# SheffieldML/GPy

Hardware: AMD Instinct MI355X
Metric: exact-GP log_lik+grad iters/sec (higher is better)
Workload: dtype f64; 1 GPU; BASELINE configs[2]: matern52 ARD exact GP, one GPRegression.parameters_changed, N=16384 D=32 Dy=1 per GPU; N=16384, D=32, kernel=matern52, ARD=True, parallelism=replicas x1

## Files before the change

### gpy_amd/csrc/kern.hip

```cpp
#include <cstdint>
#include <cstdlib>

#include "../../include/mi355gp.h"
#include "internal.h"

#define KT 64
#define KDC 32

struct CovVal {
    double k;
    double dk_r;
    double dk_or;
};

__device__ __forceinline__ double cov_k(int kind, double var, double r2, bool same = false) {
    if (kind == MI355GP_WHITE) return same ? var : 0.0;
    if (kind == MI355GP_BIAS) return var;
    if (kind == MI355GP_RBF) return var * exp(-0.5 * r2);
    const double r = sqrt(r2);
    if (kind == MI355GP_MATERN52) {
        const double s5r = 2.2360679774997896964 * r;
        return var * (1.0 + s5r + (5.0 / 3.0) * r2) * exp(-s5r);
    }
    if (kind == MI355GP_MATERN32) {
// ... 35 lines not shown
        return c;
    }
    c.k = var * exp(-r);
    c.dk_r = -r * c.k;
    c.dk_or = (r != 0.0) ? -c.k / r : 0.0;
    return c;
}

__global__ void k_scale_inputs(const double* __restrict__ X, long n, int D, const double* __restrict__ inv_ls,
                               int ard, double* __restrict__ Xt, long ldx) {
    const long idx = (long)blockIdx.x * blockDim.x + threadIdx.x;
    if (idx >= (long)D * ldx) return;
    const int q = (int)(idx / ldx);
    const long i = idx - (long)q * ldx;
    Xt[idx] = (i < n) ? X[i * D + q] * inv_ls[ard ? q : 0] : 0.0;
}

void launch_scale_inputs(hipStream_t st, const double* X, long n, int D, const double* inv_ls, int ard,
                         double* Xt, long ldx) {
    const long total = (long)D * ldx;
    hipLaunchKernelGGL(k_scale_inputs, dim3((unsigned)((total + 255) / 256)), dim3(256), 0, st, X, n, D, inv_ls,
                       ard, Xt, ldx);
}

__device__ __forceinline__ void stage_x(const double* __restrict__ Xt, long ldx, long i0, int q0, int qc,
                                        double* s, int t) {
    for (int idx = t; idx < qc * KT; idx += 256) {
        const int q = idx >> 6, ii = idx & 63;
        s[q * KT + ii] = Xt[(long)(q0 + q) * ldx + i0 + ii];
    }
}

#define KTJ 72
__device__ __forceinline__ int xj_pos(int ii) { return 40 * ((ii >> 1) & 1) + 2 * (ii >> 2) + (ii & 1); }
__device__ __forceinline__ void stage_xj(const double* __restrict__ Xt, long ldx, long i0, int q0, int qc, double* s, int t) {
    for (int idx = t; idx < qc * KT; idx += 256) {
        const int q = idx >> 6, ii = idx & 63;
        s[q * KTJ + xj_pos(ii)] = Xt[(long)(q0 + q) * ldx + i0 + ii];
    }
}
__device__ __forceinline__ d4 ld_xj(const double* sj, int q, int tx) {
    const d2 lo = *reinterpret_cast<const d2*>(sj + q * KTJ + 2 * tx);
    const d2 hi = *reinterpret_cast<const d2*>(sj + q * KTJ + 40 + 2 * tx);
    return d4{lo[0], lo[1], hi[0], hi[1]};
}

__device__ __forceinline__ void accum_r2(const double* si, const double* sj, int qc, int ty, int tx,
                                         double (&r2)[4][4]) {
    for (int q = 0; q < qc; ++q) {
        const d4 xi = *reinterpret_cast<const d4*>(si + q * KT + ty * 4);
        const d4 xj = ld_xj(sj, q, tx);
#pragma unroll
        for (int a = 0; a < 4; ++a)
#pragma unroll
            for (int b = 0; b < 4; ++b) {
                const double d = xi[a] - xj[b];
                r2[a][b] = fma(d, d, r2[a][b]);
            }
    }
}

template <bool SYM>
__global__ __launch_bounds__(256) void k_kbuild(KernParams kp, const double* __restrict__ Xt1, long ld1, long n,
                                                const double* __restrict__ Xt2, long ld2, long m,
                                                double* __restrict__ out, long ldo, long nrows_out,
                                                const double* __restrict__ noise, long noise_len, double jit,
                                                int lower_only, int add_diag, int ntc, int accumulate, int diag_same,
                                                const double* mul) {
    __shared__ __attribute__((aligned(16))) double si[KDC * KT];
    __shared__ __attribute__((aligned(16))) double sj[KDC * KTJ];
    const int t = threadIdx.x, tx = t & 15, ty = t >> 4;
    const long ti = blockIdx.x / ntc, tj = blockIdx.x % ntc;
    if (SYM && lower_only && tj > ti) return;
    const long i0 = ti * KT, j0 = tj * KT;
    double r2[4][4];
#pragma unroll
    for (int a = 0; a < 4; ++a)
#pragma unroll
        for (int b = 0; b < 4; ++b) r2[a][b] = 0.0;
    const bool real_tile = (i0 < n) && (j0 < m);
    if (real_tile) {
        for (int q0 = 0; q0 < kp.D; q0 += KDC) {
            const int qc = (kp.D - q0 < KDC) ? (kp.D - q0) : KDC;
            __syncthreads();
            stage_x(Xt1, ld1, i0, q0, qc, si, t);
            stage_xj(Xt2, ld2, j0, q0, qc, sj, t);
            __syncthreads();
            accum_r2(si, sj, qc, ty, tx, r2);
        }
    }
#pragma unroll
    for (int a = 0; a < 4; ++a) {
        const long i = i0 + ty * 4 + a;
        double v[4];
#pragma unroll
        for (int b = 0; b < 4; ++b) {
            const long j = j0 + tx * 4 + b;
            if (i < n && j < m) v[b] = cov_k(kp.kind, kp.variance, r2[a][b], (SYM || diag_same) && i == j);
            else v[b] = (SYM && i == j && !accumulate) ? 1.0 : 0.0;
        }
        if (SYM) {
            if (i < nrows_out) {
                d4* p = reinterpret_cast<d4*>(out + i * ldo + j0 + tx * 4);
                d4 o = (d4){v[0], v[1], v[2], v[3]};
                if (mul) o *= *reinterpret_cast<const d4*>(mul + i * ldo + j0 + tx * 4);
                if (add_diag && i < n) {
                    const long d = i - (j0 + tx * 4);
                    if (d >= 0 && d < 4) o[d] += noise[noise_len > 1 ? i : 0] + jit;
                }
                if (accumulate) o += *p;
                *p = o;
            }
        } else if (i < n) {
#pragma unroll
            for (int b = 0; b < 4; ++b) {
                const long j = j0 + tx * 4 + b;
                if (j < m) {
                    const double w = mul ? v[b] * mul[i * ldo + j] : v[b];
                    out[i * ldo + j] = accumulate ? out[i * ldo + j] + w : w;
                }
            }
        }
    }
}



#define KBC_DY 4
__global__ __launch_bounds__(256) void k_kbuild_cols(KernParams kp, const double* __restrict__ Xt1, long ld1, long n,
                                                     const double* __restrict__ Xt2, long ld2, long m, double* __restrict__ out,
                                                     long ldo, const double* __restrict__ V, int Dy, int ntc, int ntr,
                                                     int tiles_per_split, double* __restrict__ colpart, long mcols) {
    __shared__ __attribute__((aligned(16))) double si[KDC * KT];
    __shared__ __attribute__((aligned(16))) double sj[KDC * KTJ];
    __shared__ double sv[KT * KBC_DY];
    __shared__ double red[256];
    const int t = threadIdx.x, tx = t & 15, ty = t >> 4;
    const int tj = blockIdx.x % ntc, split = blockIdx.x / ntc;
    const long j0 = (long)tj * KT;
    const int D = kp.D;
    double csum[4][KBC_DY];
#pragma unroll
    for (int b = 0; b < 4; ++b)
#pragma unroll
        for (int d = 0; d < KBC_DY; ++d) csum[b][d] = 0.0;
    stage_xj(Xt2, ld2, j0, 0, D, sj, t);
    const bool fullcols = j0 + KT <= m;
    const int ti_end = ((split + 1) * tiles_per_split < ntr) ? (split + 1) * tiles_per_split : ntr;
    for (int ti = split * tiles_per_split; ti < ti_end; ++ti) {
        const long i0 = (long)ti * KT;
        __syncthreads();
        stage_x(Xt1, ld1, i0, 0, D, si, t);
        if (t < KT * Dy) {
            const long i = i0 + t / Dy;
            sv[(t / Dy) * KBC_DY + t % Dy] = (i < n) ? V[i * Dy + t % Dy] : 0.0;
        }
        __syncthreads();
        double r2[4][4];
#pragma unroll
        for (int a = 0; a < 4; ++a)
#pragma unroll
            for (int b = 0; b < 4; ++b) r2[a][b] = 0.0;
        accum_r2(si, sj, D, ty, tx, r2);
#pragma unroll
        for (int a = 0; a < 4; ++a) {
            const long i = i0 + ty * 4 + a;
            d4 o;
#pragma unroll
            for (int b = 0; b < 4; ++b) o[b] = (i < n && j0 + tx * 4 + b < m) ? cov_k(kp.kind, kp.variance, r2[a][b], false) : 0.0;
            if (i < n) {
                if (fullcols) *reinterpret_cast<d4*>(out + i * ldo + j0 + tx * 4) = o;
                else
#pragma unroll
                    for (int b = 0; b < 4; ++b)
                        if (j0 + tx * 4 + b < m) out[i * ldo + j0 + tx * 4 + b] = o[b];
            }
#pragma unroll
            for (int d = 0; d < KBC_DY; ++d) {
                if (d < Dy) {
                    const double v = sv[(ty * 4 + a) * KBC_DY + d];
#pragma unroll
                    for (int b = 0; b < 4; ++b) csum[b][d] = fma(o[b], v, csum[b][d]);
                }
            }
        }
    }
    double* cp = colpart + (long)split * mcols * Dy;
#pragma unroll
    for (int d = 0; d < KBC_DY; ++d) {
        if (d < Dy) {
#pragma unroll
            for (int b = 0; b < 4; ++b) {
                __syncthreads();
                red[ty * 16 + tx] = csum[b][d];
                __syncthreads();
                if (ty == 0) {
                    double sacc = 0.0;
                    for (int r = 0; r < 16; ++r) sacc += red[r * 16 + tx];
                    const long j = j0 + tx * 4 + b;
                    if (j < mcols) cp[j * Dy + d] = sacc;
                }
            }
        }
    }
}

int launch_kbuild_cols(hipStream_t st, KernParams kp, const double* Xt1, long ld1, long n, const double* Xt2, long ld2, long m,
                       long mcols, double* Kout, long ldk, const double* V, int Dy, double* colpart) {
    if (kp.D > KDC || kp.kind > MI355GP_EXPONENTIAL || Dy > KBC_DY || Dy < 1 || ldk % 4 != 0 || ((uintptr_t)Kout & 31) != 0) return 0;
    const int ntr = (int)((n + KT - 1) / KT), ntc = (int)((mcols + KT - 1) / KT);
    int nsplit = 2048 / ntc;
    if (nsplit > 64) nsplit = 64;
    if (nsplit > ntr) nsplit = ntr;
    if (nsplit < 1) nsplit = 1;
    const int tps = (ntr + nsplit - 1) / nsplit;
    nsplit = (ntr + tps - 1) / tps;
    hipLaunchKernelGGL(k_kbuild_cols, dim3((unsigned)(ntc * nsplit)), dim3(256), 0, st, kp, Xt1, ld1, n, Xt2, ld2, m, Kout, ldk, V, Dy,
                       ntc, ntr, tps, colpart, mcols);
    return nsplit;
}

static void launch_kbuild_ext(hipStream_t st, bool sym, KernParams kp, const double* Xt1, long ld1, long n, const double* Xt2,
                              long ld2, long m, double* out, long ldo, long nrows_out, const double* noise, long noise_len,
                              double jit, int lower_only, int add_diag, int ntc, int nblocks, int accumulate, int diag_same,
                              const double* mul);
static void launch_grad_ext(hipStream_t st, bool fused, KernParams kp, const double* Xt1, long ld1, long n, const double* Xt2,
                            long ld2, long m, const double* G, long ldg, const double* alpha, int Dy, long ntiles, int ntc,
                            double* partials, double* Hout, long ldh, const double* aa_scale, const double* Mul, long ldm);
static void launch_kbuild_coreg(hipStream_t st, bool sym, KernParams kp, const double* Xt1, long ld1, long n, const double* Xt2,
                                long ld2, long m, double* out, long ldo, long nrows_out, const double* noise, long noise_len,
                                double jit, int lower_only, int add_diag, int ntc, int nblocks, int accumulate, const double* mul);

static void launch_kbuild_lin(hipStream_t st, bool sym, KernParams kp, const double* Xt1, long ld1, long n, const double* Xt2,
                              long ld2, long m, double* out, long ldo, long nrows_out, const double* noise, long noise_len,
                              double jit, int lower_only, int add_diag, int ntc, int nblocks, int accumulate, const double* mul);
static void launch_grad_lin(hipStream_t st, bool fused, KernParams kp, const double* Xt1, long ld1, long n, const double* Xt2,
                            long ld2, long m, const double* G, long ldg, const double* alpha, int Dy, long ntiles, int ntc,
                            double* partials, double* Hout, long ldh, const double* aa_scale, const double* Mul, long ldm);

static inline bool dot_kind(int kind) { return kind == MI355GP_MLP || kind == MI355GP_POLY; }
static void launch_kbuild_dot(hipStream_t st, bool sym, KernParams kp, const double* Xt1, long ld1, long n, const double* Xt2,
                              long ld2, long m, double* out, long ldo, long nrows_out, const double* noise, long noise_len,
                              double jit, int lower_only, int add_diag, int ntc, int nblocks, int accumulate, const double* mul);
static void launch_grad_dot(hipStream_t st, bool fused, KernParams kp, const double* Xt1, long ld1, long n, const double* Xt2,
                            long ld2, long m, const double* G, long ldg, const double* alpha, int Dy, long ntiles, int ntc,
                            double* partials, double* Hout, long ldh, const double* aa_scale, const double* Mul, long ldm);

void launch_kbuild_sym(hipStream_t st, KernParams kp, const double* Xt, long ldx, long n, long npad, double* A,
                       const double* noise, long noise_len, double jit, int lower_only, int add_diag, int accumulate,
                       const double* mul) {
    const int nt = (int)(npad / KT);
    if (dot_kind(kp.kind)) {
        launch_kbuild_dot(st, true, kp, Xt, ldx, n, Xt, ldx, n, A, npad, npad, noise, noise_len, jit, lower_only, add_diag, nt,
                          nt * nt, accumulate, mul);
        return;
    }
    if (kp.kind == MI355GP_LINEAR) {
        launch_kbuild_lin(st, true, kp, Xt, ldx, n, Xt, ldx, n, A, npad, npad, noise, noise_len, jit, lower_only, add_diag, nt,
                          nt * nt, accumulate, mul);
        return;
    }
    if (kp.kind == MI355GP_COREGIONALIZE) {
        launch_kbuild_coreg(st, true, kp, Xt, ldx, n, Xt, ldx, n, A, npad, npad, noise, noise_len, jit, lower_only, add_diag, nt,
                            nt * nt, accumulate, mul);
        return;
    }
    if (kp.kind >= MI355GP_RATQUAD) {
        launch_kbuild_ext(st, true, kp, Xt, ldx, n, Xt, ldx, n, A, npad, npad, noise, noise_len, jit, lower_only, add_diag, nt,
                          nt * nt, accumulate, 0, mul);
        return;
    }
    hipLaunchKernelGGL((k_kbuild<true>), dim3((unsigned)((long)nt * nt)), dim3(256), 0, st, kp, Xt, ldx, n, Xt, ldx, n,
                       A, npad, npad, noise, noise_len, jit, lower_only, add_diag, nt, accumulate, 0, mul);
}

void launch_kbuild_cross(hipStream_t st, KernParams kp, const double* Xt1, long ld1, long n, const double* Xt2,
                         long ld2, long m, double* Kout, long ldk, int accumulate, int diag_same, const double* mul) {
    const int ntr = (int)((n + KT - 1) / KT), ntc = (int)((m + KT - 1) / KT);
    if (dot_kind(kp.kind)) {
        launch_kbuild_dot(st, false, kp, Xt1, ld1, n, Xt2, ld2, m, Kout, ldk, n, nullptr, 0, 0.0, 0, 0, ntc, ntr * ntc, accumulate,
                          mul);
        return;
    }
    if (kp.kind == MI355GP_LINEAR) {
        launch_kbuild_lin(st, false, kp, Xt1, ld1, n, Xt2, ld2, m, Kout, ldk, n, nullptr, 0, 0.0, 0, 0, ntc, ntr * ntc, accumulate,
                          mul);
        return;
    }
    if (kp.kind == MI355GP_COREGIONALIZE) {
        launch_kbuild_coreg(st, false, kp, Xt1, ld1, n, Xt2, ld2, m, Kout, ldk, n, nullptr, 0, 0.0, 0, 0, ntc, ntr * ntc, accumulate,
                            mul);
        return;
    }
    if (kp.kind >= MI355GP_RATQUAD) {
        launch_kbuild_ext(st, false, kp, Xt1, ld1, n, Xt2, ld2, m, Kout, ldk, n, nullptr, 0, 0.0, 0, 0, ntc, ntr * ntc,
                          accumulate, diag_same, mul);
        return;
    }
    hipLaunchKernelGGL((k_kbuild<false>), dim3((unsigned)((long)ntr * ntc)), dim3(256), 0, st, kp, Xt1, ld1, n, Xt2,
                       ld2, m, Kout, ldk, n, nullptr, 0, 0.0, 0, 0, ntc, accumulate, diag_same, mul);
}

#define GP_STRIDE 34
template <bool FUSED, bool ARD>
__global__ __launch_bounds__(256) void k_grad(KernParams kp, const double* __restrict__ Xt1, long ld1, long n,
                                              const double* __restrict__ Xt2, long ld2, long m,
                                              const double* __restrict__ G, long ldg,
                                              const double* __restrict__ alpha, int Dy, int q_off,
                                              long ntiles, int ntc, double* __restrict__ partials,
                                              double* __restrict__ Hout = nullptr, long ldh = 0, int diag_same = 0,
                                              const double* __restrict__ aa_scale = nullptr,
                                              const double* __restrict__ Mul = nullptr, long ldm = 0,
                                              RankTerm rk = RankTerm{nullptr, nullptr, 0, 0.0, 1.0, nullptr}) {
    __shared__ __attribute__((aligned(16))) double si[KDC * KT];
    __shared__ __attribute__((aligned(16))) double sj[KDC * KTJ];
    __shared__ double red[256];
    const int t = threadIdx.x, tx = t & 15, ty = t >> 4;
    double a_var = 0.0, a_iso = 0.0;
    double a_q[KDC];
#pragma unroll
    for (int q = 0; q < KDC; ++q) a_q[q] = 0.0;
    const int qcnt = ARD ? ((kp.D - q_off < KDC) ? (kp.D - q_off) : KDC) : 0;
    const double sc = (FUSED && aa_scale) ? aa_scale[0] : 1.0;

    for (long tile = blockIdx.x; tile < ntiles; tile += gridDim.x) {
        long ti, tj;
        if (FUSED) {
            ti = (long)((sqrt(8.0 * (double)tile + 1.0) - 1.0) * 0.5);
            while (ti * (ti + 1) / 2 > tile) --ti;
            while ((ti + 1) * (ti + 2) / 2 <= tile) ++ti;
            tj = tile - ti * (ti + 1) / 2;
        } else {
            ti = tile / ntc;
            tj = tile - ti * ntc;
        }
        const long i0 = ti * KT, j0 = tj * KT;
        double r2[4][4];
#pragma unroll
        for (int a = 0; a < 4; ++a)
#pragma unroll
            for (int b = 0; b < 4; ++b) r2[a][b] = 0.0;
        int last_q0 = -1;
        for (int q0 = 0; q0 < kp.D; q0 += KDC) {
            const int qc = (kp.D - q0 < KDC) ? (kp.D - q0) : KDC;
            __syncthreads();
            stage_x(Xt1, ld1, i0, q0, qc, si, t);
            stage_xj(Xt2, ld2, j0, q0, qc, sj, t);
            __syncthreads();
            accum_r2(si, sj, qc, ty, tx, r2);
            last_q0 = q0;
        }
        double gT[4][4];
#pragma unroll
        for (int a = 0; a < 4; ++a) {
            const long i = i0 + ty * 4 + a;
#pragma unroll
            for (int b = 0; b < 4; ++b) {
                const long j = j0 + tx * 4 + b;
                double g = 0.0;
                if (i < n && j < m) {
                    if (FUSED) {
                        if (j <= i) {
                            double aa = 0.0;
                            for (int d = 0; d < Dy; ++d) aa = fma(alpha[i * Dy + d], alpha[j * Dy + d], aa);
                            g = 0.5 * (sc * aa - (double)Dy * G[i * ldg + j]);
                            if (j < i) g *= 2.0;
                        }
                    } else {
                        g = G[i * ldg + j];
                        if (rk.Y) {
                            double yv = 0.0;
                            for (int d = 0; d < rk.Dy; ++d) yv = fma(rk.Y[i * rk.Dy + d], rk.V[j * rk.Dy + d], yv);
                            g = fma(rk.gscale, g, rk.beta * yv);
                            if (rk.rowscale) g *= rk.rowscale[i];
                        }
                    }
                    if (Mul) g *= Mul[i * ldm + j];
                }
                const CovVal c = cov_all(kp.kind, kp.variance, r2[a][b], (FUSED || diag_same) && i == j);
                a_var = fma(g, c.k, a_var);
                if (!ARD) a_iso = fma(g, c.dk_r, a_iso);
                gT[a][b] = g * c.dk_or;
            }
        }
        if (!FUSED && Hout) {
#pragma unroll
            for (int a = 0; a < 4; ++a) {
                const long i = i0 + ty * 4 + a;
#pragma unroll
                for (int b = 0; b < 4; ++b) {
                    const long j = j0 + tx * 4 + b;
                    if (i < n && j < m) Hout[i * ldh + j] = (r2[a][b] == 0.0) ? 0.0 : gT[a][b];
                }
            }
        }
        if (ARD) {
            if (last_q0 != q_off) {
                __syncthreads();
                stage_x(Xt1, ld1, i0, q_off, qcnt, si, t);
                stage_xj(Xt2, ld2, j0, q_off, qcnt, sj, t);
                __syncthreads();
            }
#pragma unroll
            for (int q = 0; q < KDC; ++q) {
                if (q < qcnt) {
                    const d4 xi = *reinterpret_cast<const d4*>(si + q * KT + ty * 4);
                    const d4 xj = ld_xj(sj, q, tx);
                    double s = 0.0;
#pragma unroll
                    for (int a = 0; a < 4; ++a)
#pragma unroll
                        for (int b = 0; b < 4; ++b) {
                            const double d = xi[a] - xj[b];
                            s = fma(gT[a][b], d * d, s);
                        }
                    a_q[q] += s;
                }
            }
        }
    }
    double* out = partials + (long)blockIdx.x * GP_STRIDE;
    auto block_sum = [&](double v) -> double {
        __syncthreads();
        red[t] = v;
        __syncthreads();
        for (int s = 128; s > 0; s >>= 1) {
            if (t < s) red[t] += red[t + s];
            __syncthreads();
        }
        return red[0];
    };
    const double sv = block_sum(a_var);
    if (t == 0) out[0] = sv;
    if (!ARD) {
        const double sl = block_sum(a_iso);
        if (t == 0) out[1] = sl;
    } else {
#pragma unroll
        for (int q = 0; q < KDC; ++q) {
            if (q < qcnt) {
                const double sq = block_sum(a_q[q]);
                if (t == 0) out[2 + q] = sq;
            }
        }
    }
}

static int pick_grad_blocks(long ntiles) { return (int)((ntiles < 2048) ? ntiles : 2048); }

int grad_num_blocks(long n) {
    const long nt = (n + KT - 1) / KT;
    return pick_grad_blocks(nt * (nt + 1) / 2);
}

int grad_generic_num_blocks(long n, long m) {
    return pick_grad_blocks(((n + KT - 1) / KT) * ((m + KT - 1) / KT));
}

void launch_grad_fused(hipStream_t st, KernParams kp, const double* Xt, long ldx, long n, const double* W,
                       long ldw, const double* alpha, int Dy, double* partials, int stride, const double* aa_scale,
                       const double* Mul, long ldm) {
    (void)stride;
    const long nt = (n + KT - 1) / KT;
    const long ntiles = nt * (nt + 1) / 2;
    const int nb = pick_grad_blocks(ntiles);
    if (dot_kind(kp.kind)) {
        launch_grad_dot(st, true, kp, Xt, ldx, n, Xt, ldx, n, W, ldw, alpha, Dy, ntiles, (int)nt, partials, nullptr, 0, aa_scale,
                        Mul, ldm);
        return;
    }
    if (kp.kind == MI355GP_LINEAR) {
        launch_grad_lin(st, true, kp, Xt, ldx, n, Xt, ldx, n, W, ldw, alpha, Dy, ntiles, (int)nt, partials, nullptr, 0, aa_scale,
                        Mul, ldm);
        return;
    }
    if (kp.kind >= MI355GP_RATQUAD) {
        launch_grad_ext(st, true, kp, Xt, ldx, n, Xt, ldx, n, W, ldw, alpha, Dy, ntiles, (int)nt, partials, nullptr, 0, aa_scale,
                        Mul, ldm);
        return;
    }
    if (!kp.ard) {
        hipLaunchKernelGGL((k_grad<true, false>), dim3(nb), dim3(256), 0, st, kp, Xt, ldx, n, Xt, ldx, n, W, ldw,
                           alpha, Dy, 0, ntiles, (int)nt, partials, nullptr, 0, 0, aa_scale, Mul, ldm);
    } else {
        for (int q_off = 0, gidx = 0; q_off < kp.D; q_off += KDC, ++gidx)
            hipLaunchKernelGGL((k_grad<true, true>), dim3(nb), dim3(256), 0, st, kp, Xt, ldx, n, Xt, ldx, n, W, ldw,
                               alpha, Dy, q_off, ntiles, (int)nt, partials + (long)gidx * nb * GP_STRIDE, nullptr, 0, 0,
                               aa_scale, Mul, ldm);
    }
}

#ifdef MI355GP_DIAG
template <bool ARD>
__global__ __launch_bounds__(256) void k_grad_cols(KernParams kp, const double* __restrict__ Xt1, long ld1, long n,
                                                   const double* __restrict__ Xt2, long ld2, long m,
                                                   const double* __restrict__ G, long ldg, RankTerm rk, int ntc,
                                                   int ntr, int tiles_per_split, double* __restrict__ partials,
                                                   double* __restrict__ colpart, long mcols, int nv) {
    constexpr int NVMAX = 17;
    __shared__ __attribute__((aligned(16))) double si[KDC * KT];
    __shared__ __attribute__((aligned(16))) double sj[KDC * KTJ];
    __shared__ double red[256];
    const int t = threadIdx.x, tx = t & 15, ty = t >> 4;
    const int tj = blockIdx.x % ntc, split = blockIdx.x / ntc;
    const long j0 = (long)tj * KT;
    const int D = kp.D;
    double a_var = 0.0, a_iso = 0.0;
    double a_q[NVMAX - 1];
    double hc[4][NVMAX];
#pragma unroll
    for (int q = 0; q < NVMAX - 1; ++q) a_q[q] = 0.0;
#pragma unroll
    for (int b = 0; b < 4; ++b)
#pragma unroll
        for (int c = 0; c < NVMAX; ++c) hc[b][c] = 0.0;
    const int ti_end = ((split + 1) * tiles_per_split < ntr) ? (split + 1) * tiles_per_split : ntr;
    for (int ti = split * tiles_per_split; ti < ti_end; ++ti) {
        const long i0 = (long)ti * KT;
        double r2[4][4];
#pragma unroll
        for (int a = 0; a < 4; ++a)
#pragma unroll
            for (int b = 0; b < 4; ++b) r2[a][b] = 0.0;
        __syncthreads();
        stage_x(Xt1, ld1, i0, 0, D, si, t);
        stage_xj(Xt2, ld2, j0, 0, D, sj, t);
        __syncthreads();
        accum_r2(si, sj, D, ty, tx, r2);
        double gT[4][4];
#pragma unroll
        for (int a = 0; a < 4; ++a) {
            const long i = i0 + ty * 4 + a;
#pragma unroll
            for (int b = 0; b < 4; ++b) {
                const long j = j0 + tx * 4 + b;
                double g = 0.0;
                if (i < n && j < m) {
                    g = G[i * ldg + j];
                    if (rk.Y) {
                        double yv = 0.0;
                        for (int d = 0; d < rk.Dy; ++d) yv = fma(rk.Y[i * rk.Dy + d], rk.V[j * rk.Dy + d], yv);
                        g = fma(rk.gscale, g, rk.beta * yv);
                        if (rk.rowscale) g *= rk.rowscale[i];
                    }
                }
                const CovVal c = cov_all(kp.kind, kp.variance, r2[a][b], false);
                a_var = fma(g, c.k, a_var);
                if (!ARD) a_iso = fma(g, c.dk_r, a_iso);
                gT[a][b] = g * c.dk_or;
            }
        }
#pragma unroll
        for (int q = 0; q < NVMAX - 1; ++q) {
            if (q < D) {
                const d4 xi = *reinterpret_cast<const d4*>(si + q * KT + ty * 4);
                if (ARD) {
                    const d4 xj = ld_xj(sj, q, tx);
                    double sacc = 0.0;
#pragma unroll
                    for (int a = 0; a < 4; ++a)
#pragma unroll
                        for (int b = 0; b < 4; ++b) {
                            const double d = xi[a] - xj[b];
                            sacc = fma(gT[a][b], d * d, sacc);
                        }
                    a_q[q] += sacc;
                }
#pragma unroll
                for (int b = 0; b < 4; ++b)
#pragma unroll
                    for (int a = 0; a < 4; ++a) hc[b][q] = fma(gT[a][b], xi[a], hc[b][q]);
            }
        }
#pragma unroll
        for (int b = 0; b < 4; ++b)
#pragma unroll
            for (int a = 0; a < 4; ++a) hc[b][NVMAX - 1] += gT[a][b];
    }
    double* out = partials + (long)blockIdx.x * GP_STRIDE;
    auto block_sum = [&](double v) -> double {
        __syncthreads();
        red[t] = v;
        __syncthreads();
        for (int s = 128; s > 0; s >>= 1) {
            if (t < s) red[t] += red[t + s];
            __syncthreads();
        }
        return red[0];
    };
    const double sv = block_sum(a_var);
    if (t == 0) out[0] = sv;
    if (!ARD) {
        const double sl = block_sum(a_iso);
        if (t == 0) out[1] = sl;
    } else {
#pragma unroll
        for (int q = 0; q < NVMAX - 1; ++q) {
            if (q < D) {
                const double sq = block_sum(a_q[q]);
                if (t == 0) out[2 + q] = sq;
            }
        }
    }
    double* cp = colpart + (long)split * mcols * nv;
#pragma unroll
    for (int c = 0; c < NVMAX; ++c) {
        const int cdst = (c == NVMAX - 1) ? D : c;
        if (c < D || c == NVMAX - 1) {
#pragma unroll
            for (int b = 0; b < 4; ++b) {
                __syncthreads();
                red[ty * 16 + tx] = hc[b][c];
                __syncthreads();
                if (ty == 0) {
                    double sacc = 0.0;
                    for (int r = 0; r < 16; ++r) sacc += red[r * 16 + tx];
                    const long j = j0 + tx * 4 + b;
                    if (j < mcols) cp[j * nv + cdst] = (j < m) ? sacc : 0.0;
                }
            }
        }
    }
}
#endif


#define GC_DY 4
#define GC_HS 80
template <bool ARD>
__global__ __launch_bounds__(256, 2) void k_grad_cols_mfma(KernParams kp, const double* __restrict__ Xt1, long ld1, long n,
                                                           const double* __restrict__ Xt2, long ld2, long m,
                                                           const double* __restrict__ G, long ldg, RankTerm rk, int ntc,
                                                           int ntr, int tiles_per_split, double* __restrict__ partials,
                                                           double* __restrict__ colpart, long mcols, int nv) {
    constexpr int DM = 16;
    __shared__ __attribute__((aligned(16))) double si[DM * KT];
    __shared__ __attribute__((aligned(16))) double sj[DM * KTJ];
    __shared__ __attribute__((aligned(16))) double sit[KT * 18];
    __shared__ __attribute__((aligned(16))) double sh[KT * GC_HS];
    __shared__ double red[256];
    const int t = threadIdx.x, tx = t & 15, ty = t >> 4, lane = t & 63, w = t >> 6;
    const int tj = blockIdx.x % ntc, split = blockIdx.x / ntc;
    const long j0 = (long)tj * KT;
    const int D = kp.D;
    double a_var = 0.0, a_iso = 0.0;
    double a_q[DM];
    double csum[4] = {0.0, 0.0, 0.0, 0.0};
    d4 hx = {0.0, 0.0, 0.0, 0.0};
#pragma unroll
    for (int q = 0; q < DM; ++q) a_q[q] = 0.0;
    for (int idx = t; idx < KT * 18; idx += 256) sit[idx] = 0.0;
    const bool vec4 = (j0 + tx * 4 + 3 < m) && (ldg % 4 == 0) && ((reinterpret_cast<unsigned long long>(G) & 31ull) == 0);
    const bool rkfast = rk.Y != nullptr && rk.Dy <= GC_DY;
    double vcol[4][GC_DY];
#pragma unroll
    for (int b = 0; b < 4; ++b)
#pragma unroll
        for (int d = 0; d < GC_DY; ++d)
            vcol[b][d] = (rkfast && d < rk.Dy && j0 + tx * 4 + b < m) ? rk.V[(j0 + tx * 4 + b) * rk.Dy + d] : 0.0;
    const int ti_end = ((split + 1) * tiles_per_split < ntr) ? (split + 1) * tiles_per_split : ntr;
    for (int ti = split * tiles_per_split; ti < ti_end; ++ti) {
        const long i0 = (long)ti * KT;
        double r2[4][4];
#pragma unroll
        for (int a = 0; a < 4; ++a)
#pragma unroll
            for (int b = 0; b < 4; ++b) r2[a][b] = 0.0;
        __syncthreads();
        for (int idx = t; idx < D * KT; idx += 256) {
            const int q = idx >> 6, ii = idx & 63;
            const double v = Xt1[(long)q * ld1 + i0 + ii];
            si[q * KT + ii] = v;
            sit[ii * 18 + q] = v;
        }
        stage_xj(Xt2, ld2, j0, 0, D, sj, t);
        __syncthreads();
        accum_r2(si, sj, D, ty, tx, r2);
        double gT[4][4];
#pragma unroll
        for (int a = 0; a < 4; ++a) {
            const long i = i0 + ty * 4 + a;
            d4 gv = {0.0, 0.0, 0.0, 0.0};
            double yrow[GC_DY], rs = 1.0;
            if (i < n) {
                if (vec4) gv = *reinterpret_cast<const d4*>(G + i * ldg + j0 + tx * 4);
                else
#pragma unroll
                    for (int b = 0; b < 4; ++b)
                        if (j0 + tx * 4 + b < m) gv[b] = G[i * ldg + j0 + tx * 4 + b];
                if (rk.Y && rkfast) {
#pragma unroll
                    for (int d = 0; d < GC_DY; ++d) yrow[d] = (d < rk.Dy) ? rk.Y[i * rk.Dy + d] : 0.0;
                    if (rk.rowscale) rs = rk.rowscale[i];
                }
            }
#pragma unroll
            for (int b = 0; b < 4; ++b) {
                const long j = j0 + tx * 4 + b;
                double g = 0.0;
                if (i < n && j < m) {
                    g = gv[b];
                    if (rk.Y) {
                        double yv = 0.0;
                        if (rkfast) {
#pragma unroll
                            for (int d = 0; d < GC_DY; ++d)
                                if (d < rk.Dy) yv = fma(yrow[d], vcol[b][d], yv);
                        } else {
                            for (int d = 0; d < rk.Dy; ++d) yv = fma(rk.Y[i * rk.Dy + d], rk.V[j * rk.Dy + d], yv);
                        }
                        g = fma(rk.gscale, g, rk.beta * yv);
                        if (rk.rowscale) g *= rkfast ? rs : rk.rowscale[i];
                    }
                }
                const CovVal c = cov_all(kp.kind, kp.variance, r2[a][b], false);
                a_var = fma(g, c.k, a_var);
                if (!ARD) a_iso = fma(g, c.dk_r, a_iso);
                gT[a][b] = g * c.dk_or;
                csum[b] += gT[a][b];
            }
            *reinterpret_cast<d4*>(sh + (ty * 4 + a) * GC_HS + tx * 4) = (d4){gT[a][0], gT[a][1], gT[a][2], gT[a][3]};
        }
        if (ARD) {
#pragma unroll
            for (int q = 0; q < DM; ++q) {
                if (q < D) {
                    const d4 xi = *reinterpret_cast<const d4*>(si + q * KT + ty * 4);
                    const d4 xj = ld_xj(sj, q, tx);
                    double sacc = 0.0;
#pragma unroll
                    for (int a = 0; a < 4; ++a)
#pragma unroll
                        for (int b = 0; b < 4; ++b) {
                            const double d = xi[a] - xj[b];
                            sacc = fma(gT[a][b], d * d, sacc);
                        }
                    a_q[q] += sacc;
                }
            }
        }
        __syncthreads();
        const double* ha = sh + (lane >> 4) * GC_HS + 16 * w + (lane & 15);
        const double* xb = sit + (lane >> 4) * 18 + (lane & 15);
#pragma unroll
        for (int s4 = 0; s4 < 16; ++s4) hx = mfma_f64(ha[4 * s4 * GC_HS], xb[4 * s4 * 18], hx);
    }
    double* out = partials + (long)blockIdx.x * GP_STRIDE;
    auto block_sum = [&](double v) -> double {
        __syncthreads();
        red[t] = v;
        __syncthreads();
        for (int s = 128; s > 0; s >>= 1) {
            if (t < s) red[t] += red[t + s];
            __syncthreads();
        }
        return red[0];
    };
    const double sv = block_sum(a_var);
    if (t == 0) out[0] = sv;
    if (!ARD) {
        const double sl = block_sum(a_iso);
        if (t == 0) out[1] = sl;
    } else {
#pragma unroll
        for (int q = 0; q < DM; ++q) {
            if (q < D) {
                const double sq = block_sum(a_q[q]);
                if (t == 0) out[2 + q] = sq;
            }
        }
    }
    double* cp = colpart + (long)split * mcols * nv;
#pragma unroll
    for (int r = 0; r < 4; ++r) {
        const long j = j0 + 16 * w + (lane >> 4) + 4 * r;
        const int c = lane & 15;
        if (c < D && j < mcols) cp[j * nv + c] = (j < m) ? hx[r] : 0.0;
    }
#pragma unroll
    for (int b = 0; b < 4; ++b) {
        __syncthreads();
        red[ty * 16 + tx] = csum[b];
        __syncthreads();
        if (ty == 0) {
            double sacc = 0.0;
            for (int r = 0; r < 16; ++r) sacc += red[r * 16 + tx];
            const long j = j0 + tx * 4 + b;
            if (j < mcols) cp[j * nv + D] = (j < m) ? sacc : 0.0;
        }
    }
}

int launch_grad_cols(hipStream_t st, KernParams kp, const double* Xt1, long ld1, long n, const double* Xt2, long ld2,
                     long m, long mcols, const double* G, long ldg, RankTerm rk, double* partials, double* colpart,
                     int* nblocks_out) {
    if (kp.D > 16) return 0;
    const int ntr = (int)((n + KT - 1) / KT), ntc = (int)((mcols + KT - 1) / KT);
    int nsplit = 2048 / ntc;
    if (nsplit > 64) nsplit = 64;
    if (nsplit > ntr) nsplit = ntr;
    if (nsplit < 1) nsplit = 1;
    const int tps = (ntr + nsplit - 1) / nsplit;
    nsplit = (ntr + tps - 1) / tps;
    const int nb = ntc * nsplit;
    static const int use_mfma = [] { const char* e = DIAG_ENV("GRAD_COLS_MFMA"); return (e && *e) ? atoi(e) : 1; }();
    if (use_mfma) {
        if (kp.ard)
            hipLaunchKernelGGL((k_grad_cols_mfma<true>), dim3(nb), dim3(256), 0, st, kp, Xt1, ld1, n, Xt2, ld2, m, G, ldg, rk, ntc,
                               ntr, tps, partials, colpart, mcols, kp.D + 1);
        else
            hipLaunchKernelGGL((k_grad_cols_mfma<false>), dim3(nb), dim3(256), 0, st, kp, Xt1, ld1, n, Xt2, ld2, m, G, ldg, rk, ntc,
                               ntr, tps, partials, colpart, mcols, kp.D + 1);
        *nblocks_out = nb;
        return nsplit;
    }
#ifdef MI355GP_DIAG
    if (kp.ard)
        hipLaunchKernelGGL((k_grad_cols<true>), dim3(nb), dim3(256), 0, st, kp, Xt1, ld1, n, Xt2, ld2, m, G, ldg, rk, ntc, ntr,
                           tps, partials, colpart, mcols, kp.D + 1);
    else
        hipLaunchKernelGGL((k_grad_cols<false>), dim3(nb), dim3(256), 0, st, kp, Xt1, ld1, n, Xt2, ld2, m, G, ldg, rk, ntc, ntr,
                           tps, partials, colpart, mcols, kp.D + 1);
#endif
    *nblocks_out = nb;
    return nsplit;
}

__global__ void k_studentt_scale(const double* __restrict__ scal, double nu, double n, double* __restrict__ out) {
    if (threadIdx.x == 0 && blockIdx.x == 0) out[0] = (nu + n) / (nu + scal[0] - 2.0);
}
void launch_studentt_scale(hipStream_t st, const double* scal, double nu, long n, double* out) {
    hipLaunchKernelGGL(k_studentt_scale, dim3(1), dim3(64), 0, st, scal, nu, (double)n, out);
}

void launch_grad_generic(hipStream_t st, KernParams kp, const double* Xt1, long ld1, long n, const double* Xt2,
                         long ld2, long m, int symmetric, const double* G, long ldg, double* partials,
                         int stride, double* Hout, long ldh, RankTerm rk) {
    (void)stride;
    const long ntr = (n + KT - 1) / KT, ntc = (m + KT - 1) / KT;
    const long ntiles = ntr * ntc;
    const int nb = pick_grad_blocks(ntiles);
    if (dot_kind(kp.kind)) {
        if (rk.Y) return;
        launch_grad_dot(st, false, kp, Xt1, ld1, n, Xt2, ld2, m, G, ldg, nullptr, 0, ntiles, (int)ntc, partials, Hout, ldh,
                        nullptr, nullptr, 0);
        return;
    }
    if (kp.kind == MI355GP_LINEAR) {
        if (rk.Y) return;
        launch_grad_lin(st, false, kp, Xt1, ld1, n, Xt2, ld2, m, G, ldg, nullptr, 0, ntiles, (int)ntc, partials, Hout, ldh,
                        nullptr, nullptr, 0);
        return;
    }
    if (kp.kind >= MI355GP_RATQUAD) {
        if (rk.Y) return;
        launch_grad_ext(st, false, kp, Xt1, ld1, n, Xt2, ld2, m, G, ldg, nullptr, 0, ntiles, (int)ntc, partials, Hout, ldh,
                        nullptr, nullptr, 0);
        return;
    }
    if (!kp.ard) {
        hipLaunchKernelGGL((k_grad<false, false>), dim3(nb), dim3(256), 0, st, kp, Xt1, ld1, n, Xt2, ld2, m, G, ldg,
                           nullptr, 0, 0, ntiles, (int)ntc, partials, Hout, ldh, symmetric, nullptr, nullptr, 0, rk);
    } else {
        for (int q_off = 0, gidx = 0; q_off < kp.D; q_off += KDC, ++gidx)
            hipLaunchKernelGGL((k_grad<false, true>), dim3(nb), dim3(256), 0, st, kp, Xt1, ld1, n, Xt2, ld2, m, G, ldg,
                               nullptr, 0, q_off, ntiles, (int)ntc, partials + (long)gidx * nb * GP_STRIDE,
                               (q_off + KDC >= kp.D) ? Hout : nullptr, ldh, symmetric, nullptr, nullptr, 0, rk);
    }
}

template <int NV>
__global__ __launch_bounds__(256) void k_colreduce_multi(const double* __restrict__ M, long ld, long rows, long cols,
                                                         const double* __restrict__ V, long sr, long sc, int nvt,
                                                         int nv, double* __restrict__ part, int nv_total, int c_off) {
    __shared__ double sv[NV][256];
    __shared__ double red[4][64];
    const int tx = threadIdx.x & 63, g = threadIdx.x >> 6;
    const long j = (long)blockIdx.x * 64 + tx;
    const long rs = (rows + gridDim.y - 1) / gridDim.y;
    const long r0 = (long)blockIdx.y * rs, r1 = (r0 + rs < rows) ? r0 + rs : rows;
    double acc[NV];
#pragma unroll
    for (int c = 0; c < NV; ++c) acc[c] = 0.0;
    for (long ib = r0; ib < r1; ib += 256) {
        __syncthreads();
        for (int c = 0; c < nv; ++c) {
            const long i = ib + threadIdx.x;
            sv[c][threadIdx.x] = (i < r1) ? ((c < nvt) ? V[i * sr + (long)c * sc] : 1.0) : 0.0;
        }
        __syncthreads();
        const long iend = (ib + 256 < r1) ? 256 : (r1 - ib);
        if (j < cols) {
            for (long ii = g; ii < iend; ii += 4) {
                const double x = M[(ib + ii) * ld + j];
#pragma unroll
                for (int c = 0; c < NV; ++c)
                    if (c < nv) acc[c] = fma(x, sv[c][ii], acc[c]);
            }
        }
    }
    double* out = part + ((long)blockIdx.y * cols) * nv_total + c_off;
#pragma unroll
    for (int c = 0; c < NV; ++c) {
        if (c >= nv) break;
        __syncthreads();
        red[g][tx] = acc[c];
        __syncthreads();
        if (g == 0 && j < cols) out[j * nv_total + c] = (red[0][tx] + red[1][tx]) + (red[2][tx] + red[3][tx]);
    }
}

int launch_colreduce_multi(hipStream_t st, const double* M, long ld, long rows, long cols, const double* V, long sr,
                           long sc, int nvt, int ones, double* part) {
    const int nv_total = nvt + (ones ? 1 : 0);
    int nsplit = (int)((rows + 511) / 512);
    if (nsplit < 1) nsplit = 1;
    if (nsplit > 64) nsplit = 64;
    const dim3 grid((unsigned)((cols + 63) / 64), (unsigned)nsplit);
    int c0 = 0;
    do {
        const int nvc = nvt - c0 < 32 ? nvt - c0 : 32;
        const bool lastc = c0 + nvc >= nvt;
        const int nv = nvc + ((lastc && ones) ? 1 : 0);
        const double* Vc = V + (long)c0 * sc;
        if (nv <= 9)
            hipLaunchKernelGGL((k_colreduce_multi<9>), grid, dim3(256), 0, st, M, ld, rows, cols, Vc, sr, sc, nvc, nv, part, nv_total, c0);
        else if (nv <= 17)
            hipLaunchKernelGGL((k_colreduce_multi<17>), grid, dim3(256), 0, st, M, ld, rows, cols, Vc, sr, sc, nvc, nv, part, nv_total, c0);
        else
            hipLaunchKernelGGL((k_colreduce_multi<33>), grid, dim3(256), 0, st, M, ld, rows, cols, Vc, sr, sc, nvc, nv, part, nv_total, c0);
        c0 += nvc;
    } while (c0 < nvt);
    return nsplit;
}

__global__ void k_sum_splits(const double* __restrict__ src, long cnt, int nsplit, int accumulate,
                             double* __restrict__ dst) {
    const long i = (long)blockIdx.x * blockDim.x + threadIdx.x;
    if (i >= cnt) return;
    double s = accumulate ? dst[i] : 0.0;
    for (int k = 0; k < nsplit; ++k) s += src[(long)k * cnt + i];
    dst[i] = s;
}
void launch_sum_splits(hipStream_t st, const double* src, long cnt, int nsplit, int accumulate, double* dst) {
    hipLaunchKernelGGL(k_sum_splits, dim3((unsigned)((cnt + 255) / 256)), dim3(256), 0, st, src, cnt, nsplit, accumulate,
                       dst);
}



__global__ void k_reduce_partials(const double* __restrict__ partials, int nblocks, int stride,
                                  double* __restrict__ out) {
    __shared__ double red[256];
    const int c = blockIdx.x, t = threadIdx.x;
    double s = 0.0;
    for (int b = t; b < nblocks; b += 256) s += partials[(long)b * stride + c];
    red[t] = s;
    __syncthreads();
    for (int k = 128; k > 0; k >>= 1) {
        if (t < k) red[t] += red[t + k];
        __syncthreads();
    }
    if (t == 0) out[c] = red[0];
}

void launch_reduce_partials(hipStream_t st, const double* partials, int nblocks, int stride, double* out) {
    hipLaunchKernelGGL(k_reduce_partials, dim3(stride), dim3(256), 0, st, partials, nblocks, stride, out);
}

template <int DC>
__global__ __launch_bounds__(256) void k_trmv_rows(const double* __restrict__ X, long ld, long n,
                                                   const double* __restrict__ R, int Dy, int d0,
                                                   double* __restrict__ y) {
    const int lane = threadIdx.x & 63;
    const long i = (long)blockIdx.x * 4 + (threadIdx.x >> 6);
    if (i >= n) return;
    double acc[DC];
#pragma unroll
    for (int d = 0; d < DC; ++d) acc[d] = 0.0;
    const double* xr = X + i * ld;
    long j = lane;
    for (; j + 7 * 64 <= i; j += 8 * 64) {
        double x[8];
#pragma unroll
        for (int u = 0; u < 8; ++u) x[u] = xr[j + u * 64];
#pragma unroll
        for (int u = 0; u < 8; ++u)
#pragma unroll
            for (int d = 0; d < DC; ++d)
                if (d0 + d < Dy) acc[d] = fma(x[u], R[(j + u * 64) * Dy + d0 + d], acc[d]);
    }
    for (; j <= i; j += 64) {
        const double x = xr[j];
#pragma unroll
        for (int d = 0; d < DC; ++d)
            if (d0 + d < Dy) acc[d] = fma(x, R[j * Dy + d0 + d], acc[d]);
    }
#pragma unroll
    for (int d = 0; d < DC; ++d) {
        double v = acc[d];
        for (int off = 32; off > 0; off >>= 1) v += __shfl_down(v, off);
        if (lane == 0 && d0 + d < Dy) y[i * Dy + d0 + d] = v;
    }
}

int trmv_chunk_rows(long n) { return n <= 16384 ? 64 : 256; }
template <int DC>
__global__ __launch_bounds__(256) void k_trmv_cols(const double* __restrict__ X, long ld, long n,
                                                   const double* __restrict__ y, int Dy, int d0,
                                                   double* __restrict__ part, int crows) {
    const long j = (long)blockIdx.x * 256 + threadIdx.x;
    const long c = blockIdx.y;
    const long ibeg = c * crows, iend = (ibeg + crows < n) ? ibeg + crows : n;
    if ((long)blockIdx.x * 256 >= iend) return;
    double acc[DC];
#pragma unroll
    for (int d = 0; d < DC; ++d) acc[d] = 0.0;
    if (j < n) {
        long i = ibeg;
        for (; i + 8 <= iend; i += 8) {
            double x[8];
#pragma unroll
            for (int u = 0; u < 8; ++u) x[u] = (i + u >= j) ? X[(i + u) * ld + j] : 0.0;
#pragma unroll
            for (int u = 0; u < 8; ++u)
                if (i + u >= j) {
#pragma unroll
                    for (int d = 0; d < DC; ++d)
                        if (d0 + d < Dy) acc[d] = fma(x[u], y[(i + u) * Dy + d0 + d], acc[d]);
                }
        }
        for (i = (i > j ? i : j); i < iend; ++i) {
            const double x = X[i * ld + j];
#pragma unroll
            for (int d = 0; d < DC; ++d)
                if (d0 + d < Dy) acc[d] = fma(x, y[i * Dy + d0 + d], acc[d]);
        }
#pragma unroll
        for (int d = 0; d < DC; ++d)
            if (d0 + d < Dy) part[(c * n + j) * Dy + d0 + d] = acc[d];
    }
}

__global__ void k_trmv_finish(const double* __restrict__ part, long n, int Dy, long nchunks,
                              double* __restrict__ alpha, int crows) {
    const long idx = (long)blockIdx.x * blockDim.x + threadIdx.x;
    if (idx >= n * Dy) return;
    const long j = idx / Dy;
    double s = 0.0;
    long c = j / crows;
    for (; c + 8 <= nchunks; c += 8) {
        double v[8];
#pragma unroll
        for (int u = 0; u < 8; ++u) v[u] = part[(c + u) * n * Dy + idx];
#pragma unroll
        for (int u = 0; u < 8; ++u) s += v[u];
    }
    for (; c < nchunks; ++c) s += part[c * n * Dy + idx];
    alpha[idx] = s;
}

void launch_tri_matvec(hipStream_t st, const double* X, long ld, long n, const double* R, int Dy, double* tmp,
                       double* alpha, double* partials) {
    const int crows = trmv_chunk_rows(n);
    const long nchunks = (n + crows - 1) / crows, ncolb = (n + 255) / 256;
    for (int d0 = 0; d0 < Dy; d0 += 4)
        hipLaunchKernelGGL((k_trmv_rows<4>), dim3((unsigned)((n + 3) / 4)), dim3(256), 0, st, X, ld, n, R, Dy, d0, tmp);
    for (int d0 = 0; d0 < Dy; d0 += 4)
        hipLaunchKernelGGL((k_trmv_cols<4>), dim3((unsigned)ncolb, (unsigned)nchunks), dim3(256), 0, st, X, ld, n,
                           tmp, Dy, d0, partials, crows);
    hipLaunchKernelGGL(k_trmv_finish, dim3((unsigned)((n * Dy + 255) / 256)), dim3(256), 0, st, partials, n, Dy,
                       nchunks, alpha, crows);
}

__global__ __launch_bounds__(1024) void k_scalars(const double* __restrict__ alpha, const double* __restrict__ R,
                                                  const double* __restrict__ W, long ldw, long n, int Dy,
                                                  const double* __restrict__ logsum, long nblk,
                                                  double* __restrict__ out4, double* __restrict__ diag_out,
                                                  const int* __restrict__ info) {
    __shared__ double red[4][1024];
    const int t = threadIdx.x;
    double s0 = 0.0, s1 = 0.0, s2 = 0.0, s3 = 0.0;
    for (long i = t; i < n; i += 1024) {
        double a2 = 0.0;
        for (int d = 0; d < Dy; ++d) {
            const double a = alpha[i * Dy + d];
            s0 = fma(a, R[i * Dy + d], s0);
            a2 = fma(a, a, a2);
        }
        s1 += a2;
        const double w = W ? W[i * ldw + i] : 0.0;
        s2 += w;
        if (diag_out) diag_out[i] = 0.5 * (a2 - (double)Dy * w);
    }
    for (long b = t; b < nblk; b += 1024) s3 += logsum[b];
    red[0][t] = s0; red[1][t] = s1; red[2][t] = s2; red[3][t] = s3;
    __syncthreads();
    for (int k = 512; k > 0; k >>= 1) {
        if (t < k) {
            red[0][t] += red[0][t + k]; red[1][t] += red[1][t + k];
            red[2][t] += red[2][t + k]; red[3][t] += red[3][t + k];
        }
        __syncthreads();
    }
    if (t == 0) {
        out4[0] = red[0][0]; out4[1] = red[1][0]; out4[2] = red[2][0]; out4[3] = 2.0 * red[3][0];
        if (info) out4[6] = (double)info[0];
    }
}

void launch_scalars(hipStream_t st, const double* alpha, const double* R, const double* W, long ldw, long n,
                       int Dy, const double* logsum, long nblk, double* out4, double* diag_out, const int* info) {
    hipLaunchKernelGGL(k_scalars, dim3(1), dim3(1024), 0, st, alpha, R, W, ldw, n, Dy, logsum, nblk, out4, diag_out, info);
}

__global__ void k_extract(const double* __restrict__ A, long ld, long n, int mode, const double* __restrict__ alpha,
                          int Dy, double* __restrict__ out, int transpose, const double* __restrict__ aa_scale) {
    const long nbx = (n + 255) / 256;
    const long i = blockIdx.x / nbx;
    const long j = (blockIdx.x - i * nbx) * 256 + threadIdx.x;
    if (j >= n) return;
    double v;
    if (mode == 0) {
        v = (j <= i) ? A[i * ld + j] : 0.0;
    } else {
        const long hi = i > j ? i : j, lo = i > j ? j : i;
        v = A[hi * ld + lo];
        if (mode == 2) {
            double aa = 0.0;
            for (int d = 0; d < Dy; ++d) aa = fma(alpha[i * Dy + d], alpha[j * Dy + d], aa);
            v = 0.5 * ((aa_scale ? aa_scale[0] : 1.0) * aa - (double)Dy * v);
        }
    }
    if (transpose) out[j * n + i] = v; else out[i * n + j] = v;
}

void launch_extract(hipStream_t st, const double* A, long ld, long n, int mode, const double* alpha, int Dy,
                    double* out, int transpose, const double* aa_scale) {
    hipLaunchKernelGGL(k_extract, dim3((unsigned)(((n + 255) / 256) * n)), dim3(256), 0, st, A, ld, n, mode, alpha, Dy,
                       out, transpose, aa_scale);
}

__global__ void k_pad_from_dense(const double* __restrict__ src, long n, double* __restrict__ A, long npad,
                                 const double* __restrict__ noise, long noise_len, double jit) {
    const long nbx = (npad + 255) / 256;
    const long i = blockIdx.x / nbx;
    const long j = (blockIdx.x - i * nbx) * 256 + threadIdx.x;
    if (j >= npad) return;
    double v;
    if (i < n && j < n) {
        v = src[i * n + j];
        if (i == j) v += (noise ? noise[noise_len > 1 ? i : 0] : 0.0) + jit;
    } else {
        v = (i == j) ? 1.0 : 0.0;
    }
    A[i * npad + j] = v;
}

void launch_pad_from_dense(hipStream_t st, const double* src, long n, double* A, long npad, const double* noise,
                           long noise_len, double jit) {
    hipLaunchKernelGGL(k_pad_from_dense, dim3((unsigned)(((npad + 255) / 256) * npad)), dim3(256), 0, st, src, n, A,
                       npad, noise, noise_len, jit);
}

__global__ __launch_bounds__(256) void k_col_reduce(const double* __restrict__ M, long ld, long rows, long cols,
                                                    const double* __restrict__ v, int Dy, int d, double c0, int mode,
                                                    double* __restrict__ out) {
    __shared__ double red[4][64];
    const int tx = threadIdx.x & 63, g = threadIdx.x >> 6;
    const long j = (long)blockIdx.x * 64 + tx;
// ... 1428 lines not shown
```

Baseline: 14.09 iters/s.

## Compute ARD lengthscale gradient reduction with f64 MFMA matrix form

The ARD gradient kernel gets a matrix-pipe variant. The per-dimension sum of G*(xi-xj)^2 is expanded as row-sum*xi^2 + col-sum*xj^2 - 2*xi^T G xj. The cross term runs on f64 MFMA through a transposed, centered shared-memory copy of the tile, replacing the 16-FMA-per-dimension scalar loop. It adds extra shared memory, more syncs and a new final reduction layout. The expansion also risks cancellation error, which subtracting the first point's coordinate is meant to reduce.

```diff
diff --git a/gpy_amd/csrc/kern.hip b/gpy_amd/csrc/kern.hip
--- a/gpy_amd/csrc/kern.hip
+++ b/gpy_amd/csrc/kern.hip
@@ -361,7 +361,10 @@
 }
 
 #define GP_STRIDE 34
-template <bool FUSED, bool ARD>
+#define GM_HS 68
+#define GM_XS 33
+#define GM_FS 80
+template <bool FUSED, bool ARD, bool MX = false>
 __global__ __launch_bounds__(256) void k_grad(KernParams kp, const double* __restrict__ Xt1, long ld1, long n,
                                               const double* __restrict__ Xt2, long ld2, long m,
                                               const double* __restrict__ G, long ldg,
@@ -371,15 +374,25 @@
                                               const double* __restrict__ aa_scale = nullptr,
                                               const double* __restrict__ Mul = nullptr, long ldm = 0,
                                               RankTerm rk = RankTerm{nullptr, nullptr, 0, 0.0, 1.0, nullptr}) {
-    __shared__ __attribute__((aligned(16))) double si[KDC * KT];
-    __shared__ __attribute__((aligned(16))) double sj[KDC * KTJ];
+    static_assert(!MX || ARD, "the matrix-pipe form is the ARD lengthscale reduction");
+    static_assert(KT * GM_HS == KDC * KT + KDC * KTJ && KDC * GM_FS <= KT * GM_HS, "the T tile / the final slots live in the slabs");
+    __shared__ __attribute__((aligned(32))) double sx[KDC * KT + KDC * KTJ];
+    double* const si = sx;
+    double* const sj = sx + KDC * KT;
     __shared__ double red[256];
+    __shared__ double sit[MX ? KT * GM_XS : 1];
+    __shared__ double sjt[MX ? KT * GM_XS : 1];
+    __shared__ __attribute__((aligned(32))) double srow[MX ? KT : 1];
+    __shared__ double scol[MX ? 4 * KT : 1];
     const int t = threadIdx.x, tx = t & 15, ty = t >> 4;
     double a_var = 0.0, a_iso = 0.0;
-    double a_q[KDC];
-#pragma unroll
-    for (int q = 0; q < KDC; ++q) a_q[q] = 0.0;
+    double a_q[MX ? 8 : KDC];
+#pragma unroll
+    for (int q = 0; q < (MX ? 8 : KDC); ++q) a_q[q] = 0.0;
+    double ax0 = 0.0, ax1 = 0.0;
     const int qcnt = ARD ? ((kp.D - q_off < KDC) ? (kp.D - q_off) : KDC) : 0;
+    if constexpr (MX)
+        for (int idx = t; idx < KT * GM_XS; idx += 256) sit[idx] = sjt[idx] = 0.0;
     const double sc = (FUSED && aa_scale) ? aa_scale[0] : 1.0;
 
     for (long tile = blockIdx.x; tile < ntiles; tile += gridDim.x) {
@@ -460,20 +473,79 @@
                 stage_xj(Xt2, ld2, j0, q_off, qcnt, sj, t);
                 __syncthreads();
             }
-#pragma unroll
-            for (int q = 0; q < KDC; ++q) {
-                if (q < qcnt) {
-                    const d4 xi = *reinterpret_cast<const d4*>(si + q * KT + ty * 4);
-                    const d4 xj = ld_xj(sj, q, tx);
-                    double s = 0.0;
-#pragma unroll
-                    for (int a = 0; a < 4; ++a)
-#pragma unroll
-                        for (int b = 0; b < 4; ++b) {
-                            const double d = xi[a] - xj[b];
-                            s = fma(gT[a][b], d * d, s);
-                        }
-                    a_q[q] += s;
+            if constexpr (!MX) {
+#pragma unroll
+                for (int q = 0; q < KDC; ++q) {
+                    if (q < qcnt) {
+                        const d4 xi = *reinterpret_cast<const d4*>(si + q * KT + ty * 4);
+                        const d4 xj = ld_xj(sj, q, tx);
+                        double s = 0.0;
+#pragma unroll
+                        for (int a = 0; a < 4; ++a)
+#pragma unroll
+                            for (int b = 0; b < 4; ++b) {
+                                const double d = xi[a] - xj[b];
+                                s = fma(gT[a][b], d * d, s);
+                            }
+                        a_q[q] += s;
+                    }
+                }
+            } else {
+                const int lane = t & 63, w = t >> 6;
+                for (int idx = t; idx < qcnt * KT; idx += 256) {
+                    const int q = idx >> 6, ii = idx & 63;
+                    const double c = si[q * KT];
+                    sit[ii * GM_XS + q] = si[q * KT + ii] - c;
+                    sjt[ii * GM_XS + q] = sj[q * KTJ + xj_pos(ii)] - c;
+                }
+                d4 rs;
+#pragma unroll
+                for (int a = 0; a < 4; ++a) rs[a] = (gT[a][0] + gT[a][1]) + (gT[a][2] + gT[a][3]);
+#pragma unroll
+                for (int sft = 1; sft < 16; sft <<= 1)
+#pragma unroll
+                    for (int a = 0; a < 4; ++a) rs[a] += __shfl_xor(rs[a], sft);
+                __syncthreads();
+                double* const sh = sx;
+#pragma unroll
+                for (int a = 0; a < 4; ++a)
+                    *reinterpret_cast<d4*>(sh + (ty * 4 + a) * GM_HS + tx * 4) = (d4){gT[a][0], gT[a][1], gT[a][2], gT[a][3]};
+                if (tx == 0) *reinterpret_cast<d4*>(srow + ty * 4) = rs;
+                __syncthreads();
+                {
+                    double cp = 0.0;
+#pragma unroll
+                    for (int k = 0; k < 16; ++k) cp += sh[(16 * w + k) * GM_HS + lane];
+                    scol[w * KT + lane] = cp;
+                }
+                const double* ha = sh + (lane >> 4) * GM_HS + 16 * w + (lane & 15);
+                const double* xb = sit + (lane >> 4) * GM_XS + (lane & 15);
+                const double* vj = sjt + (16 * w + (lane >> 4)) * GM_XS + (lane & 15);
+                d4 hx0 = {0.0, 0.0, 0.0, 0.0};
+                if (qcnt > 16) {
+                    d4 hx1 = {0.0, 0.0, 0.0, 0.0};
+#pragma unroll
+                    for (int s4 = 0; s4 < 16; ++s4) {
+                        const double av = ha[4 * s4 * GM_HS];
+                        hx0 = mfma_f64(av, xb[4 * s4 * GM_XS], hx0);
+                        hx1 = mfma_f64(av, xb[4 * s4 * GM_XS + 16], hx1);
+                    }
+#pragma unroll
+                    for (int r = 0; r < 4; ++r) ax1 = fma(hx1[r], vj[4 * r * GM_XS + 16], ax1);
+                } else {
+#pragma unroll
+                    for (int s4 = 0; s4 < 16; ++s4) hx0 = mfma_f64(ha[4 * s4 * GM_HS], xb[4 * s4 * GM_XS], hx0);
+                }
+#pragma unroll
+                for (int r = 0; r < 4; ++r) ax0 = fma(hx0[r], vj[4 * r * GM_XS], ax0);
+                __syncthreads();
+                const double R = srow[lane];
+                const double C = (scol[lane] + scol[KT + lane]) + (scol[2 * KT + lane] + scol[3 * KT + lane]);
+#pragma unroll
+                for (int k = 0; k < 8; ++k) {
+                    const double u = sit[lane * GM_XS + 8 * w + k], v = sjt[lane * GM_XS + 8 * w + k];
+                    a_q[k] = fma(u * u, R, a_q[k]);
+                    a_q[k] = fma(v * v, C, a_q[k]);
                 }
             }
         }
@@ -494,6 +566,24 @@
     if (!ARD) {
         const double sl = block_sum(a_iso);
         if (t == 0) out[1] = sl;
+    } else if constexpr (MX) {
+        const int lane = t & 63, w = t >> 6;
+        double* const fin = sx;
+        __syncthreads();
+#pragma unroll
+        for (int k = 0; k < 8; ++k) fin[(8 * w + k) * GM_FS + lane] = a_q[k];
+        fin[(lane & 15) * GM_FS + 64 + 4 * w + (lane >> 4)] = -2.0 * ax0;
+        fin[((lane & 15) + 16) * GM_FS + 64 + 4 * w + (lane >> 4)] = -2.0 * ax1;
+        __syncthreads();
+        double s = 0.0;
+        for (int k = 0; k < GM_FS / 8; ++k) s += fin[(t >> 3) * GM_FS + (t & 7) * (GM_FS / 8) + k];
+        red[t] = s;
+        __syncthreads();
+        if (t < qcnt) {
+            double sq = 0.0;
+            for (int p = 0; p < 8; ++p) sq += red[t * 8 + p];
+            out[2 + t] = sq;
+        }
     } else {
 #pragma unroll
         for (int q = 0; q < KDC; ++q) {
@@ -506,6 +596,12 @@
 }
 
 static int pick_grad_blocks(long ntiles) { return (int)((ntiles < 2048) ? ntiles : 2048); }
+
+#define GM_MIN_Q 9
+static bool grad_group_mfma(const KernParams& kp, int q_off) {
+    static const int use_mfma = diag_env_int(DIAG_ENV("GRAD_MFMA"), 1);
+    return use_mfma && kp.D - q_off >= GM_MIN_Q;
+}
 
 int grad_num_blocks(long n) {
     const long nt = (n + KT - 1) / KT;
@@ -542,10 +638,16 @@
         hipLaunchKernelGGL((k_grad<true, false>), dim3(nb), dim3(256), 0, st, kp, Xt, ldx, n, Xt, ldx, n, W, ldw,
                            alpha, Dy, 0, ntiles, (int)nt, partials, nullptr, 0, 0, aa_scale, Mul, ldm);
     } else {
-        for (int q_off = 0, gidx = 0; q_off < kp.D; q_off += KDC, ++gidx)
-            hipLaunchKernelGGL((k_grad<true, true>), dim3(nb), dim3(256), 0, st, kp, Xt, ldx, n, Xt, ldx, n, W, ldw,
-                               alpha, Dy, q_off, ntiles, (int)nt, partials + (long)gidx * nb * GP_STRIDE, nullptr, 0, 0,
-                               aa_scale, Mul, ldm);
+        for (int q_off = 0, gidx = 0; q_off < kp.D; q_off += KDC, ++gidx) {
+            if (grad_group_mfma(kp, q_off))
+                hipLaunchKernelGGL((k_grad<true, true, true>), dim3(nb), dim3(256), 0, st, kp, Xt, ldx, n, Xt, ldx, n, W, ldw,
+                                   alpha, Dy, q_off, ntiles, (int)nt, partials + (long)gidx * nb * GP_STRIDE, nullptr, 0, 0,
+                                   aa_scale, Mul, ldm);
+            else
+                hipLaunchKernelGGL((k_grad<true, true>), dim3(nb), dim3(256), 0, st, kp, Xt, ldx, n, Xt, ldx, n, W, ldw,
+                                   alpha, Dy, q_off, ntiles, (int)nt, partials + (long)gidx * nb * GP_STRIDE, nullptr, 0, 0,
+                                   aa_scale, Mul, ldm);
+        }
     }
 }
 
@@ -921,10 +1023,16 @@
         hipLaunchKernelGGL((k_grad<false, false>), dim3(nb), dim3(256), 0, st, kp, Xt1, ld1, n, Xt2, ld2, m, G, ldg,
                            nullptr, 0, 0, ntiles, (int)ntc, partials, Hout, ldh, symmetric, nullptr, nullptr, 0, rk);
     } else {
-        for (int q_off = 0, gidx = 0; q_off < kp.D; q_off += KDC, ++gidx)
-            hipLaunchKernelGGL((k_grad<false, true>), dim3(nb), dim3(256), 0, st, kp, Xt1, ld1, n, Xt2, ld2, m, G, ldg,
-                               nullptr, 0, q_off, ntiles, (int)ntc, partials + (long)gidx * nb * GP_STRIDE,
-                               (q_off + KDC >= kp.D) ? Hout : nullptr, ldh, symmetric, nullptr, nullptr, 0, rk);
+        for (int q_off = 0, gidx = 0; q_off < kp.D; q_off += KDC, ++gidx) {
+            if (grad_group_mfma(kp, q_off))
+                hipLaunchKernelGGL((k_grad<false, true, true>), dim3(nb), dim3(256), 0, st, kp, Xt1, ld1, n, Xt2, ld2, m, G, ldg,
+                                   nullptr, 0, q_off, ntiles, (int)ntc, partials + (long)gidx * nb * GP_STRIDE,
+                                   (q_off + KDC >= kp.D) ? Hout : nullptr, ldh, symmetric, nullptr, nullptr, 0, rk);
+            else
+                hipLaunchKernelGGL((k_grad<false, true>), dim3(nb), dim3(256), 0, st, kp, Xt1, ld1, n, Xt2, ld2, m, G, ldg,
+                                   nullptr, 0, q_off, ntiles, (int)ntc, partials + (long)gidx * nb * GP_STRIDE,
+                                   (q_off + KDC >= kp.D) ? Hout : nullptr, ldh, symmetric, nullptr, nullptr, 0, rk);
+        }
     }
 }
 
```

Measured after the change: 14.12 iters/s, median of 6. No clear change (+0.2%).
